# samuelskirvin/EIGENSOLVER

Measured on AMD Instinct MI355X. Metric: det(M) evals/sec + roots/sec, 4096x4096 (k,omega) grid, higher is better.
Workload: dtype f64

## Files before the change

eigensolver_amd/csrc/es_shoot.hip:

```cpp
#include <vector>
#include <cstdio>
#include <cstdlib>
#include <cmath>
#include <type_traits>

#include "es_shoot_shared.hpp"

namespace {
using namespace es_shoot_shared;

struct GridOpts {
  int skip;
  const int* cols;
  int part;
  int main_span;
};

constexpr long ES_TILE_GRID_X = 1L << 22;
__device__ __forceinline__ long es_tile_index() { return (long)blockIdx.y * ES_TILE_GRID_X + blockIdx.x; }
inline dim3 es_tile_grid(long tiles) {
  return tiles <= ES_TILE_GRID_X ? dim3((unsigned)tiles) : dim3((unsigned)ES_TILE_GRID_X, (unsigned)((tiles + ES_TILE_GRID_X - 1) / ES_TILE_GRID_X));
}

template <int FAM, int PTS, int MAXT, bool TRACK, int WPE = 0>
// ... 113 lines not shown
  const int lane = threadIdx.x & 63;
  double d0 = 0.0; int ok0 = 0;
  if (c < cells) { d0 = D[c]; ok0 = (st[c] == ES_PT_OK); }
  double d1 = __shfl_down(d0, 1);
  int ok1 = __shfl_down(ok0, 1);
  if (lane == 63) {
    if (c + 1 < cells) { d1 = D[c + 1]; ok1 = (st[c + 1] == ES_PT_OK); } else { d1 = 0.0; ok1 = 0; }
  }
  bool flag = false;
  if (c < cells) {
    const long row = c / nw;
    const int j = (int)(c - row * nw);
    flag = (j < nw - 1) && ok0 && ok1 && (d0 * d1 < 0.0);
  }
  const uint64_t m = __ballot(flag);
  if (lane == 0) {
    masks[c >> 6] = m;
    wave_cnt[threadIdx.x >> 6] = __popcll(m);
  }
  __syncthreads();
  if (threadIdx.x == 0) block_counts[blockIdx.x] = wave_cnt[0] + wave_cnt[1] + wave_cnt[2] + wave_cnt[3];
}

__global__ __launch_bounds__(256) void bracket_emit_kernel(const double* __restrict__ kv,
                                                           const double* __restrict__ wv, int nw, int w_mode,
                                                           long cells, const double* __restrict__ D,
                                                           const uint64_t* __restrict__ masks,
                                                           const int* __restrict__ block_off, es_root_table tab,
                                                           double* __restrict__ d_lo_sign, double* __restrict__ d_hi_sign) {
  const long c = (long)blockIdx.x * 256 + threadIdx.x;
  if (c >= cells) return;
  const uint64_t m = masks[c >> 6];
  if (!((m >> (c & 63)) & 1ull)) return;
  const int pos = es_cell_rank(masks, block_off, c);
  if (pos >= tab.capacity) return;
  const long row = c / nw;
  const int j = (int)(c - row * nw);
  const double k = kv[row];
  tab.d_k[pos] = k;
  tab.d_row[pos] = (int32_t)row;
  tab.d_w_lo[pos] = pick_w(wv, w_mode, k, (int)row, nw, j);
  tab.d_w_hi[pos] = pick_w(wv, w_mode, k, (int)row, nw, j + 1);
  d_lo_sign[pos] = D[c];
  d_hi_sign[pos] = D[c + 1];
}

constexpr int kRefineSections = 17;
constexpr int kSharedMin = 0;

constexpr int REFINE_WAVES = 4;

template <int FAM, int LANES, int CHR = 0, bool SECTIONS_ONLY = false, bool ONE = false,
          int WPE = ((FAM == FAM_CYLT || !ONE) ? 2 : 3)>
__global__ __launch_bounds__(64 * REFINE_WAVES) __attribute__((amdgpu_waves_per_eu(WPE, WPE)))
void refine_kernel(ShootDev P, es_root_table tab, double* d_lo, double* d_hi, const int* __restrict__ d_n, int n_max,
                   int n_rounds, int n_polish, double tol_percent) {
  const int n = es_count(d_n, n_max);
  if ((int)(blockIdx.x * REFINE_WAVES * (64 / LANES)) >= n) return;
  constexpr int GROUPS = 64 / LANES;
  constexpr int WTBL = GROUPS * (2 * (CHR > 0 ? CHR : 1) + 1) * FamTraits<FAM>::NE;
  __shared__ double es_point_lds[CHR > 0 ? REFINE_WAVES * WTBL : FamTraits<FAM>::NB * (2 * es_shoot_shared::CH + 1)];
  const int lane = threadIdx.x & 63;
  const int g = lane / LANES, j = lane % LANES;
  const int i = (blockIdx.x * REFINE_WAVES + ((int)threadIdx.x >> 6)) * GROUPS + g;
  const bool in = i < n;
  const double k = in ? tab.d_k[i] : 1.0;
  double lo = in ? tab.d_w_lo[i] : 1.0;
  double hi = in ? tab.d_w_hi[i] : 2.0;
  double flo = in ? d_lo[i] : 1.0;
  double fhi = in ? d_hi[i] : -1.0;
  const double frac = (double)(j + 1) / (double)(LANES + 1);
  double D = 0.0, rel = 0.0; uint8_t st = 0;
  double root = lo;
  const int n_final = (n_polish > 0) ? n_polish : (n_polish == 0 ? 1 : 0);
  const int n_it = ONE ? 1 : n_rounds + n_final;
  for (int it = 0; it < n_it; ++it) {
    const bool section = ONE ? true : it < n_rounds;
    double x;
    if (section) {
      x = lo + (hi - lo) * frac;
    } else if (n_polish > 0) {
      x = lo - flo * (hi - lo) / (fhi - flo);
      if (!(x > lo && x < hi)) x = (x == x) ? ((fabs(flo) <= fabs(fhi)) ? lo : hi) : lo + (hi - lo) * 0.5;
    } else {
      x = lo + (hi - lo) * 0.5;
    }
    if (CHR > 0) shoot_point_wavegroup<FAM, (CHR > 0 ? CHR : 1), GROUPS>(P, k, x, D, rel, st, es_point_lds + ((int)threadIdx.x >> 6) * WTBL);
    else if (SECTIONS_ONLY) shoot_point<FAM, false>(P, k, x, x, D, rel, st, es_point_lds);
    else shoot_point<FAM>(P, k, x, x, D, rel, st, es_point_lds);
    if (section) {
      const bool diff = (D * flo < 0.0);
      const unsigned long long bal = __ballot(diff);
      const unsigned long long bits = (LANES == 64) ? bal : ((bal >> (LANES * g)) & ((1ull << (LANES & 63)) - 1ull));
      const int first = bits ? (__ffsll((long long)bits) - 1) : LANES;
      const int src_hi = g * LANES + (first < LANES ? first : LANES - 1);
      const int src_lo = g * LANES + (first > 0 ? first - 1 : 0);
      const double x_hi = __shfl(x, src_hi), d_hi_new = __shfl(D, src_hi);
      const double x_lo = __shfl(x, src_lo), d_lo_new = __shfl(D, src_lo);
      if (first < LANES) { hi = x_hi; fhi = d_hi_new; }
      if (first > 0) { lo = x_lo; flo = (d_lo_new == d_lo_new) ? d_lo_new : flo; }
    } else {
      root = x;
      if (n_polish > 0) {
        if (D * flo < 0.0) { hi = x; fhi = D; } else if (D == D) { lo = x; flo = D; }
      }
    }
  }
  if (in && j == 0) {
    tab.d_w_lo[i] = lo;
    tab.d_w_hi[i] = hi;
    if (n_polish < 0) {
      d_lo[i] = flo;
      d_hi[i] = fhi;
    } else {
      tab.d_w[i] = root;
      tab.d_resid[i] = rel;
      tab.d_flag[i] = (st == ES_PT_OK && rel < tol_percent) ? 1 : 0;
    }
  }
}

template <int FAM, bool ONE = false, int WPE = ((FAM == FAM_CYLT || !ONE) ? 2 : 3)>
__global__ __launch_bounds__(64 * REFINE_WAVES) __attribute__((amdgpu_waves_per_eu(WPE, WPE)))
void refine_polish_kernel(ShootDev P, es_root_table tab, double* d_lo, double* d_hi, const int* __restrict__ d_n,
                          int n_max, int n_polish, double tol_percent) {
  ES_POINT_LDS(FAM);
  const int n = es_count(d_n, n_max);
  if ((int)(blockIdx.x * (64 * REFINE_WAVES)) >= n) return;
  const int i = blockIdx.x * (64 * REFINE_WAVES) + (int)threadIdx.x;
  const bool in = i < n;
  const double k = in ? tab.d_k[i] : 1.0;
  double lo = in ? tab.d_w_lo[i] : 1.0;
  double hi = in ? tab.d_w_hi[i] : 2.0;
  double flo = in ? d_lo[i] : 1.0;
  double fhi = in ? d_hi[i] : -1.0;
  double D = 0.0, rel = 0.0; uint8_t st = 0;
  double root = lo;
  const int n_it = ONE ? 1 : n_polish;
  for (int it = 0; it < n_it; ++it) {
    double x = lo - flo * (hi - lo) / (fhi - flo);
    if (!(x > lo && x < hi)) x = (x == x) ? ((fabs(flo) <= fabs(fhi)) ? lo : hi) : lo + (hi - lo) * 0.5;
    shoot_point<FAM>(P, k, x, x, D, rel, st, es_point_lds);
    root = x;
    if (D * flo < 0.0) { hi = x; fhi = D; } else if (D == D) { lo = x; flo = D; }
  }
  if (in) {
    tab.d_w_lo[i] = lo;
    tab.d_w_hi[i] = hi;
    if (ONE && n_polish == 0) {
      d_lo[i] = flo;
      d_hi[i] = fhi;
    } else {
      tab.d_w[i] = root;
      tab.d_resid[i] = rel;
      tab.d_flag[i] = (st == ES_PT_OK && rel < tol_percent) ? 1 : 0;
    }
  }
}

constexpr int kHybridSections = 1;
constexpr int kHybridSteps = 8;
constexpr double kHybridEps = 1e-12;

struct HybridState {
  double* lo; double* hi; double* flo; double* fhi; double* xprev;
  int* info;
};
constexpr int HYB_ACTIVE = 0, HYB_KEPT = 1, HYB_FAILED = 2;

template <int FAM, int WPE = (FAM == FAM_CYL0 ? 3 : 2)>
__global__ __launch_bounds__(64 * REFINE_WAVES) __attribute__((amdgpu_waves_per_eu(WPE, WPE)))
void refine_superlinear_kernel(ShootDev P, es_root_table tab, const double* d_lo, const double* d_hi, HybridState S,
                               const int* __restrict__ d_n, int n_max, int step, double tol_percent,
                               unsigned long long* stats) {
  ES_POINT_LDS(FAM);
  const int n = es_count(d_n, n_max);
  if ((int)(blockIdx.x * (64 * REFINE_WAVES)) >= n) return;
  const int i = blockIdx.x * (64 * REFINE_WAVES) + (int)threadIdx.x;
  const bool in = i < n;
  const bool first = step == 0;
  const int info = (in && !first) ? S.info[i] : 0;
  const bool active = in && ((info >> 2) == HYB_ACTIVE);
  if (!__syncthreads_or(active ? 1 : 0)) return;
  const double k = in ? tab.d_k[i] : 1.0;
  double lo, hi, flo, fhi, xprev;
  if (first) {
    lo = in ? tab.d_w_lo[i] : 1.0;
    hi = in ? tab.d_w_hi[i] : 2.0;
    flo = in ? d_lo[i] : 1.0;
    fhi = in ? d_hi[i] : -1.0;
    xprev = NAN;
  } else {
    lo = active ? S.lo[i] : 1.0;
    hi = active ? S.hi[i] : 2.0;
    flo = active ? S.flo[i] : 1.0;
    fhi = active ? S.fhi[i] : -1.0;
    xprev = active ? S.xprev[i] : NAN;
  }
  int side = info & 3, status = info >> 2;
  double D = 0.0, rel = 0.0; uint8_t st = 0;
  double x = lo - flo * (hi - lo) / (fhi - flo);
  if (!(x > lo && x < hi)) x = lo + (hi - lo) * 0.5;
  shoot_point<FAM>(P, k, x, x, D, rel, st, es_point_lds);
  if (active) {
    if (D == D) {
      if (D * flo < 0.0) { hi = x; fhi = D; if (side == 1) flo *= 0.5; side = 1; }
      else { lo = x; flo = D; if (side == 2) fhi *= 0.5; side = 2; }
      const double ax = fabs(x);
      if (D == 0.0 || fabs(x - xprev) <= kHybridEps * ax || (hi - lo) <= kHybridEps * ax)
        status = (st == ES_PT_OK && rel < tol_percent) ? HYB_KEPT : HYB_FAILED;
    } else {
      status = HYB_FAILED;
    }
    if (status == HYB_KEPT) {
      tab.d_w_lo[i] = lo;
      tab.d_w_hi[i] = hi;
      tab.d_w[i] = x;
      tab.d_resid[i] = rel;
      tab.d_flag[i] = 1;
    } else if (status == HYB_ACTIVE) {
      S.lo[i] = lo; S.hi[i] = hi; S.flo[i] = flo; S.fhi[i] = fhi; S.xprev[i] = x;
    }
    S.info[i] = side | (status << 2);
  }
  const int n_eval = __popcll(__ballot(active)), n_kept = __popcll(__ballot(active && status == HYB_KEPT));
  if ((threadIdx.x & 63) == 0) {
    if (first && n_eval) atomicAdd(stats + 0, (unsigned long long)n_eval);
    if (n_kept) atomicAdd(stats + 1, (unsigned long long)n_kept);
    if (n_eval) atomicAdd(stats + 3, (unsigned long long)n_eval);
  }
}

__global__ __launch_bounds__(256) void hybrid_flag_kernel(const int* __restrict__ info, const int* __restrict__ d_n,
                                                          int n_max, uint64_t* __restrict__ masks,
                                                          int* __restrict__ block_counts, unsigned long long* stats) {
  __shared__ int wave_cnt[4];
  const int n = es_count(d_n, n_max);
  const int i = blockIdx.x * 256 + (int)threadIdx.x;
  const bool flag = i < n && (info[i] >> 2) != HYB_KEPT;
  const uint64_t m = __ballot(flag);
  if ((threadIdx.x & 63) == 0) {
    masks[i >> 6] = m;
    wave_cnt[threadIdx.x >> 6] = __popcll(m);
  }
  __syncthreads();
  if (threadIdx.x == 0) {
    const int c = wave_cnt[0] + wave_cnt[1] + wave_cnt[2] + wave_cnt[3];
    block_counts[blockIdx.x] = c;
    if (c) atomicAdd(stats + 2, (unsigned long long)c);
  }
}

__global__ __launch_bounds__(256) void hybrid_gather_kernel(es_root_table tab, es_root_table ftab, int* __restrict__ idx,
                                                            const uint64_t* __restrict__ masks,
                                                            const int* __restrict__ block_off,
                                                            const int* __restrict__ d_n, int n_max) {
  const int n = es_count(d_n, n_max);
  const int i = blockIdx.x * 256 + (int)threadIdx.x;
  if (i >= n) return;
  if (!((masks[i >> 6] >> (i & 63)) & 1ull)) return;
  const int pos = es_cell_rank(masks, block_off, (long)i);
  if (pos >= ftab.capacity) return;
  ftab.d_k[pos] = tab.d_k[i];
  ftab.d_w_lo[pos] = tab.d_w_lo[i];
  ftab.d_w_hi[pos] = tab.d_w_hi[i];
  ftab.d_w[pos] = tab.d_w[i];
  ftab.d_resid[pos] = tab.d_resid[i];
  ftab.d_row[pos] = tab.d_row[i];
  idx[pos] = i;
}

__global__ __launch_bounds__(256) void hybrid_scatter_kernel(es_root_table ftab, es_root_table tab,
                                                             const int* __restrict__ idx,
                                                             const int* __restrict__ d_nf, int n_max) {
  const int nf = *d_nf < n_max ? *d_nf : n_max;
  const int j = blockIdx.x * 256 + (int)threadIdx.x;
  if (j >= nf) return;
  const int i = idx[j];
  if (i < 0 || i >= tab.capacity) return;
  tab.d_w[i] = ftab.d_w[j];
  tab.d_w_lo[i] = ftab.d_w_lo[j];
  tab.d_w_hi[i] = ftab.d_w_hi[j];
  tab.d_resid[i] = ftab.d_resid[j];
  tab.d_flag[i] = ftab.d_flag[j];
}

constexpr float F32_TAU_NODE = 1e-3f;
constexpr double F32_TAU_D = 5e-2;
constexpr double F32_TAU_POLE = 5e-2;
constexpr uint8_t F32_UNSURE = 0x80;

typedef float v2f __attribute__((ext_vector_type(2)));

__device__ __forceinline__ v2f v2(float x) { return (v2f){x, x}; }
__device__ __forceinline__ v2f vfma(v2f a, v2f b, v2f c) { return __builtin_elementwise_fma(a, b, c); }
__device__ __forceinline__ v2f vabs(v2f a) { return __builtin_elementwise_abs(a); }
__device__ __forceinline__ v2f vmin(v2f a, v2f b) { return __builtin_elementwise_min(a, b); }
__device__ __forceinline__ v2f vmax(v2f a, v2f b) { return __builtin_elementwise_max(a, b); }
__device__ __forceinline__ v2f vrcp(v2f a) { return (v2f){__builtin_amdgcn_rcpf(a.x), __builtin_amdgcn_rcpf(a.y)}; }

struct CoefF { v2f a11, a12, a21, a22; };
struct CoefPreF { v2f n11, n12, n21, n22, den; };

template <bool TRACK>
struct ScreenF {
  v2f mn = {3.0e38f, 3.0e38f};
// ... 480 lines not shown
GridShape pick_shape(int nw, bool track) {
  GridShape best{4, 2};
  double best_cost = 1e300;
  for (int pts : {4, 3, 2, 1}) {
    if (ShapeTable<FAM>::wpe[pts] == 0) continue;
    const int T = shape_threads(nw, pts);
    const long span = (long)T * pts;
    const long padded = (nw + span - 1) / span * span;
    static const double wave_count_cost[5] = {0.0, 1.83, 1.39, 1.17, 1.0};
    const double c = (double)padded * ShapeTable<FAM>::cost[pts] * wave_count_cost[T / 64];
    if (c < best_cost) { best_cost = c; best = GridShape{pts, ShapeTable<FAM>::wpe[pts]}; }
  }
  if (track && fam_has_bands<FAM>()) best.wpe = 2;
  if (const char* ev = getenv("ES_GRID_SHAPE")) {
    int p = 0, w = 0;
    if (sscanf(ev, "%d,%d", &p, &w) == 2 && p >= 1 && p <= 4 && w >= 2 && w <= 4) best = GridShape{p, w};
  }
  return best;
}

template <int FAM, int PTS, int WPE, bool TRACK>
constexpr bool shape_built() {
  if (PTS == 3 && ShapeTable<FAM>::wpe[3] == 0) return false;
#if defined(ES_ALL_GRID_SHAPES)
  return true;
#else
  if (TRACK && fam_has_bands<FAM>()) return WPE == 2;
  if (FAM == FAM_CYL0 && PTS == 4 && WPE == 2) return true;
  return ShapeTable<FAM>::wpe[PTS] == WPE;
#endif
}

template <int FAM>
bool rows2_shape(int nw, bool track) {
  if (!fam_has_bands<FAM>() || track || nw > 512) return false;
  const char* r2 = getenv("ES_GRID_ROWS2");
  return !(r2 && r2[0] == '0') && !getenv("ES_GRID_SHAPE");
}

template <int FAM>
int launch_grid(es_context* ctx, const es_problem* prob, const double* d_k, int nk, const double* d_w, int nw,
                int w_mode, double* d_D, double* d_rel, uint8_t* d_status, int flags = 0) {
  GridOpts opts;
  opts.skip = (flags & ES_EVAL_SKIP_CONTINUUM) ? 1 : 0;
  opts.cols = nullptr;
  opts.part = 0;
  opts.main_span = 0;
  if (opts.skip && w_mode == ES_W_PHASE_SPEED && fam_has_bands<FAM>() && prob->dev.use_bands) {
    if ((size_t)nw + 1 > ctx->cols_cap) {
      ES_HIP_CHECK(ctx, hipStreamSynchronize(ctx->stream));
      if (ctx->d_cols) ES_HIP_CHECK(ctx, hipFree(ctx->d_cols));
      if (ctx->d_coldead) ES_HIP_CHECK(ctx, hipFree(ctx->d_coldead));
      ctx->d_cols = nullptr; ctx->d_coldead = nullptr; ctx->cols_cap = 0;
      ES_HIP_CHECK(ctx, hipMalloc(&ctx->d_cols, ((size_t)nw + 1) * sizeof(int)));
      ES_HIP_CHECK(ctx, hipMalloc(&ctx->d_coldead, (size_t)nw));
      ctx->cols_cap = (size_t)nw + 1;
    }
    hipLaunchKernelGGL(column_classify_kernel, dim3(1), dim3(1024), 0, ctx->stream, prob->dev, d_w, nw, ctx->d_cols,
                       ctx->d_coldead);
    ES_HIP_CHECK(ctx, hipGetLastError());
    const long cells = (long)nk * nw;
    const int fb = (int)((cells + 255) / 256 < 8192 ? (cells + 255) / 256 : 8192);
    hipLaunchKernelGGL(fill_dead_columns_kernel, dim3(fb), dim3(256), 0, ctx->stream, prob->dev, d_k, nk, d_w, nw,
                       ctx->d_coldead, d_D, d_rel, d_status);
    ES_HIP_CHECK(ctx, hipGetLastError());
    opts.cols = ctx->d_cols;
  }
  const bool track = !(fam_has_bands<FAM>() && prob->dev.use_bands);
  GridShape shape = pick_shape<FAM>(nw, track);
  const int T = shape_threads(nw, shape.pts);
  const long tiles = (long)nk * ((nw + (long)T * shape.pts - 1) / ((long)T * shape.pts));
  const dim3 grid = es_tile_grid(tiles);
  bool launched = false;
  es_timer_begin(ctx);
  if constexpr (fam_has_bands<FAM>()) {
    if (rows2_shape<FAM>(nw, track) && !opts.cols && nk >= 2) {
      const int pts2 = (nw + 127) / 128;
      const dim3 grid2 = es_tile_grid(((long)nk + 1) / 2);
#define ES_R2(P_)                                                                                                   \
      if (pts2 == P_) hipLaunchKernelGGL((shoot_grid_kernel_r2<FAM, P_, false, 3>), grid2, dim3(256), 0, ctx->stream, \
                                         prob->dev, d_k, nk, d_w, nw, w_mode, d_D, d_rel, d_status, opts);
      ES_R2(1) ES_R2(2) ES_R2(3) ES_R2(4)
#undef ES_R2
      launched = true;
    }
  }
  auto one = [&](auto pts_c, auto wpe_c, auto track_c) {
    constexpr int PTS = decltype(pts_c)::value, WPE = decltype(wpe_c)::value;
    constexpr bool TRACK = decltype(track_c)::value;
    if constexpr (shape_built<FAM, PTS, WPE, TRACK>() && (TRACK || fam_has_bands<FAM>())) {
      if (launched || shape.pts != PTS || shape.wpe != WPE || track != TRACK) return;
      launched = true;
      if constexpr (FAM == FAM_CYL0 && PTS == 4 && !TRACK) {
        if (opts.cols && T > 64) {
          opts.part = 1;
          hipLaunchKernelGGL((shoot_grid_kernel<FAM, PTS, 256, TRACK, WPE>), grid, dim3(T), 0, ctx->stream,
                             prob->dev, d_k, nk, d_w, nw, w_mode, d_D, d_rel, d_status, opts);
          opts.part = 2;
          opts.main_span = 4 * T;
          const long tiles2 = (long)nk * (T / 64);
          hipLaunchKernelGGL((shoot_grid_kernel<FAM, 4, 64, false, 2>), es_tile_grid(tiles2),
                             dim3(64), 0, ctx->stream, prob->dev, d_k, nk, d_w, nw, w_mode, d_D, d_rel, d_status, opts);
          return;
        }
      }
      hipLaunchKernelGGL((shoot_grid_kernel<FAM, PTS, 256, TRACK, WPE>), grid, dim3(T), 0, ctx->stream, prob->dev,
                         d_k, nk, d_w, nw, w_mode, d_D, d_rel, d_status, opts);
    }
  };
  using std::integral_constant;
#define ES_SHAPE(P_, W_)                                                                                            \
  one(integral_constant<int, P_>{}, integral_constant<int, W_>{}, integral_constant<bool, false>{});                \
  one(integral_constant<int, P_>{}, integral_constant<int, W_>{}, integral_constant<bool, true>{});
  ES_SHAPE(4, 2) ES_SHAPE(4, 3) ES_SHAPE(4, 4) ES_SHAPE(3, 2) ES_SHAPE(3, 3) ES_SHAPE(2, 2) ES_SHAPE(2, 3) ES_SHAPE(2, 4) ES_SHAPE(1, 2) ES_SHAPE(1, 3) ES_SHAPE(1, 4)
#undef ES_SHAPE
  es_timer_end(ctx);
  if (!launched) {
    ctx->last_error = "grid launch shape not built (ES_GRID_SHAPE names a shape outside this build)";
    return ES_ERR_UNSUPPORTED;
  }
  ES_HIP_CHECK(ctx, hipGetLastError());
  return ES_SUCCESS;
}

inline int es_bound(long n_max) { return (int)(n_max < INT32_MAX ? n_max : INT32_MAX); }
inline dim3 es_blocks(long n_max) { return dim3((unsigned)((n_max + 255) / 256)); }

template <int FAM>
int launch_points(es_context* ctx, const es_problem* prob, const double* d_k, const double* d_w, const int* d_n, long n_max,
                  double* d_D, double* d_rel, uint8_t* d_status) {
  hipLaunchKernelGGL((shoot_points_kernel<FAM>), es_blocks(n_max), dim3(256), 0, ctx->stream, prob->dev, d_k, d_w, d_n,
                     es_bound(n_max), d_D, d_rel, d_status);
  ES_HIP_CHECK(ctx, hipGetLastError());
  return ES_SUCCESS;
}

int dispatch_points(es_context* ctx, const es_problem* prob, const double* d_k, const double* d_w, const int* d_n, long n_max,
                    double* d_D, double* d_rel, uint8_t* d_status) {
#define CALL_PTS(F) launch_points<F>(ctx, prob, d_k, d_w, d_n, n_max, d_D, d_rel, d_status)
  ES_DISPATCH_FAMILY(prob->dev.family, CALL_PTS)
#undef CALL_PTS
}

template <int FAM>
int launch_refine_steps(es_context* ctx, const es_problem* prob, const es_root_table& tab, double* d_lo, double* d_hi,
                        const int* d_n, int n_max, int n_hint, int sections, int rounds, int np, bool polish, double tol) {
  constexpr int CHR = (FAM == FAM_CYL0) ? 32 : 0;
  int shared_min = kSharedMin;
  if (const char* ev = getenv("ES_REFINE_SHARED_MIN")) shared_min = atoi(ev);
  const bool shared_entries = CHR > 0 && np < 0 && n_hint >= shared_min && !getenv("ES_REFINE_PRIVATE_ENTRIES");
  auto blocks = [&](int per_wg) { return dim3((n_max + per_wg - 1) / per_wg); };
  constexpr bool ONE_ROUND_FAM = (FAM == FAM_CYLT || FAM == FAM_CYL0);
  const bool one_round = ONE_ROUND_FAM && !getenv("ES_REFINE_ROUNDS_IN_KERNEL");
#define ES_REFINE(LANES_, CHR_, SO_, PER_WG_)                                                                           \
  if (SO_ && one_round) {                                                                                               \
    if constexpr (ONE_ROUND_FAM && SO_) {                                                                               \
      for (int r_ = 0; r_ < rounds; ++r_)                                                                               \
        hipLaunchKernelGGL((refine_kernel<FAM, LANES_, CHR_, true, true>), blocks(PER_WG_), dim3(64 * REFINE_WAVES), 0, \
                           ctx->stream, prob->dev, tab, d_lo, d_hi, d_n, n_max, 1, np, tol);                            \
    }                                                                                                                   \
  } else                                                                                                                \
    hipLaunchKernelGGL((refine_kernel<FAM, LANES_, CHR_, SO_, false>), blocks(PER_WG_), dim3(64 * REFINE_WAVES), 0,     \
                       ctx->stream, prob->dev, tab, d_lo, d_hi, d_n, n_max, rounds, np, tol)
  if (sections == 17 && shared_entries) ES_REFINE(16, CHR, true, 4 * REFINE_WAVES);
  else if (np < 0) {
    if (sections == 17) ES_REFINE(16, 0, true, 4 * REFINE_WAVES);
    else if (sections == 9) ES_REFINE(8, 0, true, 8 * REFINE_WAVES);
    else ES_REFINE(4, 0, true, 16 * REFINE_WAVES);
  } else {
    if (sections == 17) ES_REFINE(16, 0, false, 4 * REFINE_WAVES);
    else if (sections == 9) ES_REFINE(8, 0, false, 8 * REFINE_WAVES);
    else ES_REFINE(4, 0, false, 16 * REFINE_WAVES);
  }
#undef ES_REFINE
  ES_HIP_CHECK(ctx, hipGetLastError());
  if (np < 0 && polish) {
    if (one_round) {
      if constexpr (ONE_ROUND_FAM) {
        for (int p_ = 0; p_ < ES_REFINE_POLISH; ++p_)
          hipLaunchKernelGGL((refine_polish_kernel<FAM, true>), blocks(64 * REFINE_WAVES), dim3(64 * REFINE_WAVES), 0, ctx->stream,
                             prob->dev, tab, d_lo, d_hi, d_n, n_max, p_ == ES_REFINE_POLISH - 1 ? 1 : 0, tol);
      }
    } else
      hipLaunchKernelGGL((refine_polish_kernel<FAM, false>), blocks(64 * REFINE_WAVES), dim3(64 * REFINE_WAVES), 0, ctx->stream,
                         prob->dev, tab, d_lo, d_hi, d_n, n_max, ES_REFINE_POLISH, tol);
    ES_HIP_CHECK(ctx, hipGetLastError());
  }
  return ES_SUCCESS;
}

int refine_sections() {
  int sections = kRefineSections;
  if (const char* ev = getenv("ES_REFINE_SECTIONS")) {
    const int v = atoi(ev);
    if (v == 5 || v == 9 || v == 17) sections = v;
  }
  return sections;
}

int check_refine_rule(es_context* ctx) {
  if (ctx->refine_rule == ES_REFINE_HYBRID && refine_sections() != kRefineSections) {
    ctx->last_error = "ES_REFINE_HYBRID is defined for 17-section only (ES_REFINE_SECTIONS is set to another rule)";
    return ES_ERR_UNSUPPORTED;
  }
  return ES_SUCCESS;
}

template <int FAM>
int launch_refine_hybrid(es_context* ctx, const es_problem* prob, const es_root_table& tab, const int* d_n, int n_max,
                         int n_hint, int rounds, double tol) {
  if (n_max <= 0) return ES_SUCCESS;
  auto align = [](size_t b) { return (b + 255) & ~(size_t)255; };
  const size_t cap = (size_t)n_max;
  const size_t bd = align(cap * sizeof(double)), bi = align(cap * sizeof(int)), bf = align(cap);
  const int nblk = (n_max + 255) / 256;
  const size_t bm = align((size_t)nblk * 4 * sizeof(uint64_t)), bc = align((size_t)(nblk + 1) * sizeof(int));
  int rc = es_ensure_hybrid_scratch(ctx, 10 * bd + 3 * bi + bf + bm + bc + 256);
  if (rc) return rc;
  char* b = (char*)ctx->d_hybrid;
  auto take = [&](size_t bytes) { char* p = b; b += bytes; return p; };
  HybridState S;
  S.lo = (double*)take(bd); S.hi = (double*)take(bd); S.flo = (double*)take(bd); S.fhi = (double*)take(bd);
  S.xprev = (double*)take(bd);
  S.info = (int*)take(bi);
  es_root_table ftab;
  ftab.d_k = (double*)take(bd); ftab.d_w = (double*)take(bd); ftab.d_w_lo = (double*)take(bd);
  ftab.d_w_hi = (double*)take(bd); ftab.d_resid = (double*)take(bd);
  ftab.d_row = (int32_t*)take(bi); ftab.d_flag = (uint8_t*)take(bf);
  ftab.capacity = n_max;
  int* idx = (int*)take(bi);
  uint64_t* masks = (uint64_t*)take(bm);
  int* counts = (int*)take(bc);
  int* d_nf = (int*)take(256);
  rc = launch_refine_steps<FAM>(ctx, prob, tab, tab.d_w, tab.d_resid, d_n, n_max, n_hint, kRefineSections, kHybridSections,
                                -1, false, tol);
  if (rc) return rc;
  const dim3 wg(64 * REFINE_WAVES), grid((n_max + 64 * REFINE_WAVES - 1) / (64 * REFINE_WAVES));
  for (int s_ = 0; s_ < kHybridSteps; ++s_)
    hipLaunchKernelGGL((refine_superlinear_kernel<FAM>), grid, wg, 0, ctx->stream, prob->dev, tab, tab.d_w, tab.d_resid, S,
                       d_n, n_max, s_, tol, ctx->d_refine_stats);
  ES_HIP_CHECK(ctx, hipGetLastError());
  hipLaunchKernelGGL(hybrid_flag_kernel, dim3(nblk), dim3(256), 0, ctx->stream, S.info, d_n, n_max, masks, counts,
                     ctx->d_refine_stats);
  ES_HIP_CHECK(ctx, hipGetLastError());
  rc = es_scan_counts_async(ctx, counts, nblk, d_nf);
  if (rc) return rc;
  hipLaunchKernelGGL(hybrid_gather_kernel, dim3(nblk), dim3(256), 0, ctx->stream, tab, ftab, idx, masks, counts, d_n, n_max);
  ES_HIP_CHECK(ctx, hipGetLastError());
  rc = launch_refine_steps<FAM>(ctx, prob, ftab, ftab.d_w, ftab.d_resid, d_nf, n_max, n_hint, kRefineSections,
                                rounds - kHybridSections, -1, true, tol);
  if (rc) return rc;
  hipLaunchKernelGGL(hybrid_scatter_kernel, dim3(nblk), dim3(256), 0, ctx->stream, ftab, tab, idx, d_nf, n_max);
  ES_HIP_CHECK(ctx, hipGetLastError());
  return ES_SUCCESS;
}

template <int FAM>
int launch_refine(es_context* ctx, const es_problem* prob, const es_root_table& tab, double* d_lo, double* d_hi,
                  const int* d_n, int n_max, int n_hint, int n_bisect, double tol) {
  const int sections = refine_sections();
  int rounds = 0;
  for (double span = 1.0, need = ldexp(1.0, n_bisect < 1000 ? n_bisect : 1000); span < need; span *= (double)sections) ++rounds;
  if (ctx->refine_rule == ES_REFINE_HYBRID) {
    const int rc = check_refine_rule(ctx);
    if (rc) return rc;
    if (rounds > kHybridSections) return launch_refine_hybrid<FAM>(ctx, prob, tab, d_n, n_max, n_hint, rounds, tol);
  }
  const int np = (ES_REFINE_POLISH > 0 && rounds > 0) ? -1 : ES_REFINE_POLISH;
  return launch_refine_steps<FAM>(ctx, prob, tab, d_lo, d_hi, d_n, n_max, n_hint, sections, rounds, np, true, tol);
}

int dispatch_refine(es_context* ctx, const es_problem* prob, const es_root_table& tab, const int* d_n, int n_max, int n_hint,
                    int n_bisect, double tol) {
#define CALL_REFINE(F) launch_refine<F>(ctx, prob, tab, tab.d_w, tab.d_resid, d_n, n_max, n_hint, n_bisect, tol)
  ES_DISPATCH_FAMILY(prob->dev.family, CALL_REFINE)
#undef CALL_REFINE
}

}

extern "C" int es_problem_create(es_context* ctx, const es_shoot_desc* d, const es_profiles* pr, es_problem** out) {
  if (!ctx) return ES_ERR_INVALID_ARG;
  ES_REQUIRE(ctx, d && pr && out, "null pointer");
  *out = nullptr;
  ES_REQUIRE(ctx, d->n_nodes >= 2 && d->n_nodes <= (1 << 24), "n_nodes out of range");
  ES_REQUIRE(ctx, d->geometry >= 0 && d->geometry <= 3, "geometry");
  ES_REQUIRE(ctx, d->x_boundary == -1.0 || d->x_boundary == 1.0, "x_boundary must be -1 or +1");
  const int N = d->n_nodes, npts = 2 * N - 1;
  int nb = 0;
  switch (d->geometry) {
    case ES_GEOM_CYLINDER: nb = FamTraits<FAM_CYL0>::NB; break;
    case ES_GEOM_CYLINDER_TWIST: nb = FamTraits<FAM_CYLT>::NB; break;
    case ES_GEOM_SLAB_DENSITY: nb = FamTraits<FAM_SLABD>::NB; break;
    default: nb = FamTraits<FAM_SLABF>::NB; break;
  }
  std::vector<double> base((size_t)nb * npts);
  auto B = [&](int f, int i) -> double& { return base[(size_t)f * npts + i]; };
  if (d->geometry == ES_GEOM_CYLINDER || d->geometry == ES_GEOM_CYLINDER_TWIST) {
    ES_REQUIRE(ctx, pr->r && pr->rho && pr->c2 && pr->Bz, "cylinder profiles r, rho, c2, Bz required");
    ES_REQUIRE(ctx, d->axis_bc >= 0 && d->axis_bc <= 2, "axis_bc");
    ES_REQUIRE(ctx, d->c1_power == 1 || d->c1_power == 2, "c1_power");
    ES_REQUIRE(ctx, d->m >= 0 && d->m_ext >= 0 && d->m_ext <= 64, "m");
    for (int i = 0; i < npts; ++i) {
      const double r = pr->r[i], rho = pr->rho[i], c2 = pr->c2[i], Bz = pr->Bz[i];
      const double Bphi = pr->Bphi ? pr->Bphi[i] : 0.0;
      const double vz = pr->vz ? pr->vz[i] : 0.0;
      const double vphi = pr->vphi ? pr->vphi[i] : 0.0;
      const double sr = sqrt(rho);
      const double bA = Bz / sr;
      const double vA = (Bz + Bphi) / sr;
      const double S = c2 + vA * vA;
      const double q = c2 / S;
      if (d->geometry == ES_GEOM_CYLINDER) {
        ES_REQUIRE(ctx, Bphi == 0.0 && vphi == 0.0, "ES_GEOM_CYLINDER needs Bphi = vphi = 0 (use CYLINDER_TWIST)");
        B(C0_VZ, i) = vz;
        B(C0_BA, i) = bA;
        B(C0_Q, i) = q;
        B(C0_A1, i) = rho / r;
        B(C0_B1, i) = r / (rho * S);
        B(C0_E1, i) = 1.0 / (r * rho);
        B(C0_E2, i) = r / rho;
      } else {
        const double dm = (double)d->m, dm2 = dm * dm;
        const double invr = 1.0 / r, invr2 = invr * invr;
        const double bphr = Bphi / r, vphr = vphi / r;
        const double Bphi_n = bphr * r, vphi_n = vphr * r;
        B(CT_MB, i) = dm * bphr;
        B(CT_BZ, i) = Bz;
        B(CT_BA, i) = bA;
        B(CT_MV, i) = dm * vphr;
        B(CT_VZ, i) = vz;
// ... 593 lines not shown
```

eigensolver_amd/csrc/es_shoot_shared.hpp:

```cpp
#pragma once
#include "es_common.hpp"
#include "es_shoot_device.hpp"

struct es_problem {
  ShootDev dev;
  double* d_base = nullptr;
  es_shoot_desc desc;
};

namespace es_shoot_shared {

constexpr int ES_REFINE_POLISH = 2;
#if defined(ES_STAGE_FAR_NODE_ALWAYS)
#define ES_FAR_NODE(c_, n_) 1
#else
#define ES_FAR_NODE(c_, n_) (((c_) == (n_) - 1) ? 1 : 0)
#endif
constexpr int CH = 128;

template <int FAM>
__device__ __forceinline__ void load_base(const ShootDev& P, int pt, double* b) {
#pragma unroll
  for (int f = 0; f < FamTraits<FAM>::NB; ++f) b[f] = P.base[(size_t)f * P.npts + pt];
}
// ... 88 lines not shown
          Coef Nm, N1, Nm2, N2;
          ES_ENTRY(2 * j - 3, e)
          ES_ENTRY(2 * j - 4, e1)
          ES_ENTRY(2 * j - 5, em2)
          ES_ENTRY(2 * j - 6, e2)
          coefficients4<FAM, TRACK>(e, e1, em2, e2, P, s, w, Nm, N1, Nm2, N2, trk);
          adjoint_step<FAM>(zp, zq, B0, Cm, C1, h, h2, h6, h3);
          adjoint_step<FAM>(zp, zq, C1, Cm2, C2, h, h2, h6, h3);
          B0 = C2;
          Cm = Nm; C1 = N1; Cm2 = Nm2; C2 = N2;
        }
        adjoint_step<FAM>(zp, zq, B0, Cm, C1, h, h2, h6, h3);
        adjoint_step<FAM>(zp, zq, C1, Cm2, C2, h, h2, h6, h3);
        B0 = C2;
      }
    } else {
      Coef Cm, C1;
      ES_ENTRY(2 * j + 1, e)
      ES_ENTRY(2 * j, e2)
      coefficients2<FAM, TRACK, C1P>(e, e2, P, s, w, Cm, C1, trk);
      for (; j >= 1; --j) {
        Coef Nm, N1;
        ES_ENTRY(2 * j - 1, e)
        ES_ENTRY(2 * j - 2, e2)
        coefficients2<FAM, TRACK, C1P>(e, e2, P, s, w, Nm, N1, trk);
        adjoint_step<FAM>(zp, zq, B0, Cm, C1, h, h2, h6, h3);
        B0 = C1;
        Cm = Nm; C1 = N1;
      }
      adjoint_step<FAM>(zp, zq, B0, Cm, C1, h, h2, h6, h3);
      B0 = C1;
    }
#undef ES_ENTRY
    adjoint_rescale<FAM>(zp, zq, nsteps - c0 - nst, nsteps - c0);
  }
  const Mismatch M = boundary_algebra<FAM>(P, s, w, X, zp, zq, e2);
  finish_point(P, M, X, TRACK ? trk.crossed() : (BANDS ? band_crossed(P, k, w) : false), D, rel, st);
}

template <int FAM, bool TRACK, int CHR, int NG>
__device__ __forceinline__ void shoot_point_wavegroup_impl(const ShootDev& P, double k, double w, double& D, double& rel,
                                                           uint8_t& st, double* __restrict__ tbl) {
  constexpr int NE = FamTraits<FAM>::NE;
  constexpr int NB = FamTraits<FAM>::NB;
  constexpr int NODES = 2 * CHR + 1;
  constexpr int GL = 64 / NG;
  const int lane = threadIdx.x & 63;
  const int grp = lane / GL;
  const KScal s = make_kscal(P, k);
  const int nsteps = P.n_nodes - 1;
  const double h = P.h, h2 = 0.5 * P.h, h6 = P.h / 6.0, h3 = P.h / 3.0;
  SignTrack trk;
  double e[NE], e2[NE];
  const ExteriorLite X = exterior_lite(P, k, w, w);
  Coef B0;
  double zp = 0.0, zq = 0.0;
  const double* mine = tbl + (size_t)grp * NODES * NE;
  double kgs[NG];
#pragma unroll
  for (int g2 = 0; g2 < NG; ++g2) kgs[g2] = __shfl(k, g2 * GL);
  const int nchunks = (nsteps + CHR - 1) / CHR;
  for (int c = nchunks - 1; c >= 0; --c) {
    const int c0 = c * CHR;
    const int nst = (nsteps - c0 < CHR) ? (nsteps - c0) : CHR;
    const int nn = 2 * nst + ES_FAR_NODE(c, nchunks);
    __builtin_amdgcn_wave_barrier();
    for (int idx = lane; idx < NG * nn; idx += 64) {
      const int g2 = idx / nn, i = idx - g2 * nn;
      double kg = kgs[0];
#pragma unroll
      for (int q = 1; q < NG; ++q) kg = (g2 == q) ? kgs[q] : kg;
      const KScal sg = make_kscal(P, kg);
      double b[NB], eg[NE];
#pragma unroll
      for (int f = 0; f < NB; ++f) b[f] = P.base[(size_t)f * P.npts + 2 * c0 + i];
      make_entry<FAM, fam_scaled<FAM>()>(b, sg, eg);
#pragma unroll
      for (int f = 0; f < NE; ++f) tbl[((size_t)g2 * NODES + i) * NE + f] = eg[f];
    }
    __builtin_amdgcn_wave_barrier();
    if (c == nchunks - 1) {
#pragma unroll
      for (int f = 0; f < NE; ++f) e[f] = mine[2 * nst * NE + f];
      coefficients<FAM, TRACK>(e, P, s, w, B0, trk);
      adjoint_start(P, B0, zp, zq);
    }
    int j = nst - 1;
    if (!fam_rcp4<FAM>() || !(j & 1)) {
      for (; j >= 0 && (!fam_rcp4<FAM>() || !(j & 1)); --j) {
        Coef Bm, B1;
#pragma unroll
        for (int f = 0; f < NE; ++f) { e[f] = mine[(2 * j + 1) * NE + f]; e2[f] = mine[2 * j * NE + f]; }
        coefficients2<FAM, TRACK>(e, e2, P, s, w, Bm, B1, trk);
        adjoint_step<FAM>(zp, zq, B0, Bm, B1, h, h2, h6, h3);
        B0 = B1;
      }
    }
    if (fam_rcp4<FAM>() && j >= 1) {
      double e1[NE], em2[NE];
      Coef Cm, C1, Cm2, C2;
#pragma unroll
      for (int f = 0; f < NE; ++f) {
        e[f] = mine[(2 * j + 1) * NE + f]; e1[f] = mine[2 * j * NE + f];
        em2[f] = mine[(2 * j - 1) * NE + f]; e2[f] = mine[(2 * j - 2) * NE + f];
      }
      coefficients4<FAM, TRACK>(e, e1, em2, e2, P, s, w, Cm, C1, Cm2, C2, trk);
      for (; j >= 3; j -= 2) {
        Coef Nm, N1, Nm2, N2;
#pragma unroll
        for (int f = 0; f < NE; ++f) {
          e[f] = mine[(2 * j - 3) * NE + f]; e1[f] = mine[(2 * j - 4) * NE + f];
          em2[f] = mine[(2 * j - 5) * NE + f]; e2[f] = mine[(2 * j - 6) * NE + f];
        }
        coefficients4<FAM, TRACK>(e, e1, em2, e2, P, s, w, Nm, N1, Nm2, N2, trk);
        adjoint_step<FAM>(zp, zq, B0, Cm, C1, h, h2, h6, h3);
        adjoint_step<FAM>(zp, zq, C1, Cm2, C2, h, h2, h6, h3);
        B0 = C2;
        Cm = Nm; C1 = N1; Cm2 = Nm2; C2 = N2;
      }
      adjoint_step<FAM>(zp, zq, B0, Cm, C1, h, h2, h6, h3);
      adjoint_step<FAM>(zp, zq, C1, Cm2, C2, h, h2, h6, h3);
      B0 = C2;
    }
    adjoint_rescale<FAM>(zp, zq, nsteps - c0 - nst, nsteps - c0);
  }
  const Mismatch M = boundary_algebra<FAM>(P, s, w, X, zp, zq, e2);
  finish_point(P, M, X, TRACK ? trk.crossed() : band_crossed(P, k, w), D, rel, st);
}

template <int FAM, int CHR, int NG>
__device__ __forceinline__ void shoot_point_wavegroup(const ShootDev& P, double k, double w, double& D, double& rel,
                                                      uint8_t& st, double* __restrict__ tbl) {
  if (fam_has_bands<FAM>() && P.use_bands) shoot_point_wavegroup_impl<FAM, !fam_has_bands<FAM>(), CHR, NG>(P, k, w, D, rel, st, tbl);
  else shoot_point_wavegroup_impl<FAM, true, CHR, NG>(P, k, w, D, rel, st, tbl);
}

template <int FAM, bool STATUS = true>
__device__ __forceinline__ void shoot_point(const ShootDev& P, double k, double w, double w_cst, double& D,
                                            double& rel, uint8_t& st, double* __restrict__ sb) {
  if (FAM == FAM_CYLT) {
    if (!STATUS) {
      if (P.c1_power == 2) shoot_point_impl<FAM, false, false, 2>(P, k, w, w_cst, D, rel, st, sb);
      else shoot_point_impl<FAM, false, false, 1>(P, k, w, w_cst, D, rel, st, sb);
    } else {
      if (P.c1_power == 2) shoot_point_impl<FAM, true, false, 2>(P, k, w, w_cst, D, rel, st, sb);
      else shoot_point_impl<FAM, true, false, 1>(P, k, w, w_cst, D, rel, st, sb);
    }
  } else if (!STATUS) {
    shoot_point_impl<FAM, false, false>(P, k, w, w_cst, D, rel, st, sb);
  } else if (fam_has_bands<FAM>() && P.use_bands) shoot_point_impl<FAM, !fam_has_bands<FAM>()>(P, k, w, w_cst, D, rel, st, sb);
  else shoot_point_impl<FAM, true>(P, k, w, w_cst, D, rel, st, sb);
}

#define ES_POINT_LDS(FAM) __shared__ double es_point_lds[FamTraits<FAM>::NB * (2 * es_shoot_shared::CH + 1)]

}
```

Before: 855.2 million.

## Add copy-free paired-march refine and secant kernels for CYL0 family

For the CYL0 family, the per-round refine and polish launches now go to new kernels. These use a paired adjoint march with double-buffered coefficient sets (coefficients4, steps unrolled by four) and read node entries directly from a wave-shared LDS table rather than copying them into private arrays. The round kernel brackets the sign change using a ballot and shuffle across the section lanes. The aim is to cut register and copy overhead in the shooting march. In exchange there is more code and register pressure, and bracket selection and rescaling may differ slightly from the legacy path.

```diff
diff --git a/eigensolver_amd/csrc/es_shoot.hip b/eigensolver_amd/csrc/es_shoot.hip
--- a/eigensolver_amd/csrc/es_shoot.hip
+++ b/eigensolver_amd/csrc/es_shoot.hip
@@ -289,6 +289,88 @@
       d_hi[i] = fhi;
     } else {
       tab.d_w[i] = root;
+      tab.d_resid[i] = rel;
+      tab.d_flag[i] = (st == ES_PT_OK && rel < tol_percent) ? 1 : 0;
+    }
+  }
+}
+
+template <int FAM, int LANES, int CHR, int WPE = 3>
+__global__ __launch_bounds__(64 * REFINE_WAVES) __attribute__((amdgpu_waves_per_eu(WPE, WPE)))
+void section_round_kernel(ShootDev P, es_root_table tab, double* d_lo, double* d_hi, const int* __restrict__ d_n, int n_max) {
+  static_assert(CHR > 0 && 64 % LANES == 0 && LANES < 64, "wave-shared node entries");
+  const int n = es_count(d_n, n_max);
+  if ((int)(blockIdx.x * REFINE_WAVES * (64 / LANES)) >= n) return;
+  constexpr int GROUPS = 64 / LANES;
+  constexpr int WTBL = GROUPS * (2 * CHR + 1) * FamTraits<FAM>::NE;
+  __shared__ double es_point_lds[REFINE_WAVES * WTBL];
+  const int lane = threadIdx.x & 63;
+  const int g = lane / LANES, j = lane % LANES;
+  const int i = (blockIdx.x * REFINE_WAVES + ((int)threadIdx.x >> 6)) * GROUPS + g;
+  const bool in = i < n;
+  const double k = in ? tab.d_k[i] : 1.0;
+  double x;
+  {
+    const double lo0 = in ? tab.d_w_lo[i] : 1.0, hi0 = in ? tab.d_w_hi[i] : 2.0;
+    x = lo0 + (hi0 - lo0) * ((double)(j + 1) / (double)(LANES + 1));
+  }
+  double D = 0.0, rel = 0.0; uint8_t st = 0;
+  shoot_point_wavegroup_impl2<FAM, false, CHR, GROUPS>(P, k, x, D, rel, st, es_point_lds + ((int)threadIdx.x >> 6) * WTBL);
+  __asm__ volatile("" ::: "memory");
+  double lo = in ? tab.d_w_lo[i] : 1.0;
+  double hi = in ? tab.d_w_hi[i] : 2.0;
+  double flo = in ? d_lo[i] : 1.0;
+  double fhi = in ? d_hi[i] : -1.0;
+  const bool diff = (D * flo < 0.0);
+  const unsigned long long bal = __ballot(diff);
+  const unsigned long long bits = (bal >> (LANES * g)) & ((1ull << LANES) - 1ull);
+  const int first = bits ? (__ffsll((long long)bits) - 1) : LANES;
+  const int src_hi = g * LANES + (first < LANES ? first : LANES - 1);
+  const int src_lo = g * LANES + (first > 0 ? first - 1 : 0);
+  const double x_hi = __shfl(x, src_hi), d_hi_new = __shfl(D, src_hi);
+  const double x_lo = __shfl(x, src_lo), d_lo_new = __shfl(D, src_lo);
+  if (first < LANES) { hi = x_hi; fhi = d_hi_new; }
+  if (first > 0) { lo = x_lo; flo = (d_lo_new == d_lo_new) ? d_lo_new : flo; }
+  if (in && j == 0) {
+    tab.d_w_lo[i] = lo;
+    tab.d_w_hi[i] = hi;
+    d_lo[i] = flo;
+    d_hi[i] = fhi;
+  }
+}
+
+template <int FAM, int WPE = 3>
+__global__ __launch_bounds__(64 * REFINE_WAVES) __attribute__((amdgpu_waves_per_eu(WPE, WPE)))
+void secant_step_kernel(ShootDev P, es_root_table tab, double* d_lo, double* d_hi, const int* __restrict__ d_n, int n_max,
+                        int last, double tol_percent) {
+  ES_POINT_LDS(FAM);
+  const int n = es_count(d_n, n_max);
+  if ((int)(blockIdx.x * (64 * REFINE_WAVES)) >= n) return;
+  const int i = blockIdx.x * (64 * REFINE_WAVES) + (int)threadIdx.x;
+  const bool in = i < n;
+  const double k = in ? tab.d_k[i] : 1.0;
+  double lo = in ? tab.d_w_lo[i] : 1.0;
+  double hi = in ? tab.d_w_hi[i] : 2.0;
+  double flo = in ? d_lo[i] : 1.0;
+  double fhi = in ? d_hi[i] : -1.0;
+  double D = 0.0, rel = 0.0; uint8_t st = 0;
+  double x = lo - flo * (hi - lo) / (fhi - flo);
+  if (!(x > lo && x < hi)) x = (x == x) ? ((fabs(flo) <= fabs(fhi)) ? lo : hi) : lo + (hi - lo) * 0.5;
+  shoot_point2<FAM>(P, k, x, x, D, rel, st, es_point_lds);
+  __asm__ volatile("" ::: "memory");
+  lo = in ? tab.d_w_lo[i] : 1.0;
+  hi = in ? tab.d_w_hi[i] : 2.0;
+  flo = in ? d_lo[i] : 1.0;
+  fhi = in ? d_hi[i] : -1.0;
+  if (D * flo < 0.0) { hi = x; fhi = D; } else if (D == D) { lo = x; flo = D; }
+  if (in) {
+    tab.d_w_lo[i] = lo;
+    tab.d_w_hi[i] = hi;
+    if (!last) {
+      d_lo[i] = flo;
+      d_hi[i] = fhi;
+    } else {
+      tab.d_w[i] = x;
       tab.d_resid[i] = rel;
       tab.d_flag[i] = (st == ES_PT_OK && rel < tol_percent) ? 1 : 0;
     }
@@ -1075,9 +1157,20 @@
   auto blocks = [&](int per_wg) { return dim3((n_max + per_wg - 1) / per_wg); };
   constexpr bool ONE_ROUND_FAM = (FAM == FAM_CYLT || FAM == FAM_CYL0);
   const bool one_round = ONE_ROUND_FAM && !getenv("ES_REFINE_ROUNDS_IN_KERNEL");
+  constexpr bool COPY_FREE_FAM = (FAM == FAM_CYL0);
+  const char* march_ev = getenv("ES_REFINE_MARCH");
+  const bool copy_free = COPY_FREE_FAM && one_round && !(march_ev && !strcmp(march_ev, "legacy"));
 #define ES_REFINE(LANES_, CHR_, SO_, PER_WG_)                                                                           \
   if (SO_ && one_round) {                                                                                               \
-    if constexpr (ONE_ROUND_FAM && SO_) {                                                                               \
+    if constexpr (COPY_FREE_FAM && SO_ && CHR_ > 0) {                                                                   \
+      for (int r_ = 0; r_ < rounds; ++r_)                                                                               \
+        if (copy_free)                                                                                                  \
+          hipLaunchKernelGGL((section_round_kernel<FAM, LANES_, CHR_>), blocks(PER_WG_), dim3(64 * REFINE_WAVES), 0,    \
+                             ctx->stream, prob->dev, tab, d_lo, d_hi, d_n, n_max);                                      \
+        else                                                                                                            \
+          hipLaunchKernelGGL((refine_kernel<FAM, LANES_, CHR_, true, true>), blocks(PER_WG_), dim3(64 * REFINE_WAVES),  \
+                             0, ctx->stream, prob->dev, tab, d_lo, d_hi, d_n, n_max, 1, np, tol);                       \
+    } else if constexpr (ONE_ROUND_FAM && SO_) {                                                                        \
       for (int r_ = 0; r_ < rounds; ++r_)                                                                               \
         hipLaunchKernelGGL((refine_kernel<FAM, LANES_, CHR_, true, true>), blocks(PER_WG_), dim3(64 * REFINE_WAVES), 0, \
                            ctx->stream, prob->dev, tab, d_lo, d_hi, d_n, n_max, 1, np, tol);                            \
@@ -1099,7 +1192,15 @@
   ES_HIP_CHECK(ctx, hipGetLastError());
   if (np < 0 && polish) {
     if (one_round) {
-      if constexpr (ONE_ROUND_FAM) {
+      if constexpr (COPY_FREE_FAM) {
+        for (int p_ = 0; p_ < ES_REFINE_POLISH; ++p_)
+          if (copy_free)
+            hipLaunchKernelGGL((secant_step_kernel<FAM>), blocks(64 * REFINE_WAVES), dim3(64 * REFINE_WAVES), 0, ctx->stream,
+                               prob->dev, tab, d_lo, d_hi, d_n, n_max, p_ == ES_REFINE_POLISH - 1 ? 1 : 0, tol);
+          else
+            hipLaunchKernelGGL((refine_polish_kernel<FAM, true>), blocks(64 * REFINE_WAVES), dim3(64 * REFINE_WAVES), 0, ctx->stream,
+                               prob->dev, tab, d_lo, d_hi, d_n, n_max, p_ == ES_REFINE_POLISH - 1 ? 1 : 0, tol);
+      } else if constexpr (ONE_ROUND_FAM) {
         for (int p_ = 0; p_ < ES_REFINE_POLISH; ++p_)
           hipLaunchKernelGGL((refine_polish_kernel<FAM, true>), blocks(64 * REFINE_WAVES), dim3(64 * REFINE_WAVES), 0, ctx->stream,
                              prob->dev, tab, d_lo, d_hi, d_n, n_max, p_ == ES_REFINE_POLISH - 1 ? 1 : 0, tol);
diff --git a/eigensolver_amd/csrc/es_shoot_shared.hpp b/eigensolver_amd/csrc/es_shoot_shared.hpp
--- a/eigensolver_amd/csrc/es_shoot_shared.hpp
+++ b/eigensolver_amd/csrc/es_shoot_shared.hpp
@@ -264,6 +264,183 @@
   else shoot_point_impl<FAM, true>(P, k, w, w_cst, D, rel, st, sb);
 }
 
+#define ES_PAIRED_MARCH(LOAD4)                                                                 \
+  if (j >= 1) {                                                                                \
+    double e1[NE], em2[NE];                                                                    \
+    Coef Am, A1, Am2, A2, Bm, B1, Bm2, B2;                                                     \
+    LOAD4(j)                                                                                   \
+    coefficients4<FAM, TRACK>(e, e1, em2, e2, P, s, w, Am, A1, Am2, A2, trk);                  \
+    if (((j + 1) >> 1) & 1) {                           \
+      if (j >= 3) {                                                                            \
+        LOAD4(j - 2)                                                                           \
+        coefficients4<FAM, TRACK>(e, e1, em2, e2, P, s, w, Bm, B1, Bm2, B2, trk);              \
+      }                                                                                        \
+      adjoint_step<FAM>(zp, zq, B0, Am, A1, h, h2, h6, h3);                                    \
+      adjoint_step<FAM>(zp, zq, A1, Am2, A2, h, h2, h6, h3);                                   \
+      B0 = A2;                                                                                 \
+      if (j >= 3) { Am = Bm; A1 = B1; Am2 = Bm2; A2 = B2; }    \
+      j -= 2;                                                                                  \
+    }                                                                                          \
+    for (; j >= 7; j -= 4) {                            \
+      LOAD4(j - 2)                                                                             \
+      coefficients4<FAM, TRACK>(e, e1, em2, e2, P, s, w, Bm, B1, Bm2, B2, trk);                \
+      adjoint_step<FAM>(zp, zq, B0, Am, A1, h, h2, h6, h3);                                    \
+      adjoint_step<FAM>(zp, zq, A1, Am2, A2, h, h2, h6, h3);                                   \
+      B0 = A2;                                                                                 \
+      LOAD4(j - 4)                                                                             \
+      coefficients4<FAM, TRACK>(e, e1, em2, e2, P, s, w, Am, A1, Am2, A2, trk);                \
+      adjoint_step<FAM>(zp, zq, B0, Bm, B1, h, h2, h6, h3);                                    \
+      adjoint_step<FAM>(zp, zq, B1, Bm2, B2, h, h2, h6, h3);                                   \
+      B0 = B2;                                                                                 \
+    }                                                                                          \
+    if (j >= 3) {                                                      \
+      LOAD4(j - 2)                                                                             \
+      coefficients4<FAM, TRACK>(e, e1, em2, e2, P, s, w, Bm, B1, Bm2, B2, trk);                \
+      adjoint_step<FAM>(zp, zq, B0, Am, A1, h, h2, h6, h3);                                    \
+      adjoint_step<FAM>(zp, zq, A1, Am2, A2, h, h2, h6, h3);                                   \
+      adjoint_step<FAM>(zp, zq, A2, Bm, B1, h, h2, h6, h3);                                    \
+      adjoint_step<FAM>(zp, zq, B1, Bm2, B2, h, h2, h6, h3);                                   \
+      B0 = B2;                                                                                 \
+    }                                                                                          \
+  }
+
+template <int FAM, bool TRACK, bool BANDS = !TRACK>
+__device__ __forceinline__ void shoot_point_impl2(const ShootDev& P, double k, double w, double w_cst, double& D,
+                                                  double& rel, uint8_t& st, double* __restrict__ sb) {
+  static_assert(fam_rcp4<FAM>(), "paired marches only");
+  constexpr int NE = FamTraits<FAM>::NE;
+  constexpr int NB = FamTraits<FAM>::NB;
+  const KScal s = make_kscal(P, k);
+  const int nsteps = P.n_nodes - 1;
+  const double h = P.h, h2 = 0.5 * P.h, h6 = P.h / 6.0, h3 = P.h / 3.0;
+  SignTrack trk;
+  double b[NB], e[NE], e2[NE];
+  const ExteriorLite X = exterior_lite(P, k, w, w_cst);
+  Coef B0;
+  double zp = 0.0, zq = 0.0;
+  const int nchunks = (nsteps + CH - 1) / CH;
+  for (int c = nchunks - 1; c >= 0; --c) {
+    const int c0 = c * CH;
+    const int nst = (nsteps - c0 < CH) ? (nsteps - c0) : CH;
+    __syncthreads();
+#pragma unroll
+    for (int f = 0; f < NB; ++f)
+      for (int i = threadIdx.x; i < 2 * nst + ES_FAR_NODE(c, nchunks); i += blockDim.x)
+        sb[i * NB + f] = P.base[(size_t)f * P.npts + 2 * c0 + i];
+    __syncthreads();
+#define ES_ENTRY(NODE, E)                                                                      \
+    {                                                                                          \
+      _Pragma("unroll") for (int f = 0; f < NB; ++f) b[f] = sb[(NODE) * NB + f];               \
+      make_entry<FAM, fam_scaled<FAM>()>(b, s, E);                                             \
+    }
+#define ES_ENTRY4(J) ES_ENTRY(2 * (J) + 1, e) ES_ENTRY(2 * (J), e1) ES_ENTRY(2 * (J) - 1, em2) ES_ENTRY(2 * (J) - 2, e2)
+    if (c == nchunks - 1) {
+      ES_ENTRY(2 * nst, e)
+      coefficients<FAM, TRACK>(e, P, s, w, B0, trk);
+      adjoint_start(P, B0, zp, zq);
+    }
+    int j = nst - 1;
+    if (!(j & 1)) {
+      Coef Bm, B1;
+      ES_ENTRY(2 * j + 1, e)
+      ES_ENTRY(2 * j, e2)
+      coefficients2<FAM, TRACK>(e, e2, P, s, w, Bm, B1, trk);
+      adjoint_step<FAM>(zp, zq, B0, Bm, B1, h, h2, h6, h3);
+      B0 = B1;
+      --j;
+    }
+    ES_PAIRED_MARCH(ES_ENTRY4)
+#undef ES_ENTRY4
+#undef ES_ENTRY
+    adjoint_rescale<FAM>(zp, zq, nsteps - c0 - nst, nsteps - c0);
+  }
+  const Mismatch M = boundary_algebra<FAM>(P, s, w, X, zp, zq, e2);
+  finish_point(P, M, X, TRACK ? trk.crossed() : (BANDS ? band_crossed(P, k, w) : false), D, rel, st);
+}
+
+template <int FAM, bool TRACK, int CHR, int NG>
+__device__ __forceinline__ void shoot_point_wavegroup_impl2(const ShootDev& P, double k, double w, double& D, double& rel,
+                                                            uint8_t& st, double* __restrict__ tbl) {
+  static_assert(fam_rcp4<FAM>() && CHR % 2 == 0, "paired marches only");
+  constexpr int NE = FamTraits<FAM>::NE;
+  constexpr int NB = FamTraits<FAM>::NB;
+  constexpr int NODES = 2 * CHR + 1;
+  constexpr int GL = 64 / NG;
+  const int lane = threadIdx.x & 63;
+  const int grp = lane / GL;
+  const KScal s = make_kscal(P, k);
+  const int nsteps = P.n_nodes - 1;
+  const double h = P.h, h2 = 0.5 * P.h, h6 = P.h / 6.0, h3 = P.h / 3.0;
+  SignTrack trk;
+  double e[NE], e2[NE];
+  Coef B0;
+  double zp = 0.0, zq = 0.0;
+  const double* mine = tbl + (size_t)grp * NODES * NE;
+  double kgs[NG];
+#pragma unroll
+  for (int g2 = 0; g2 < NG; ++g2)
+    kgs[g2] = __hiloint2double(__builtin_amdgcn_readlane(__double2hiint(k), g2 * GL),
+                               __builtin_amdgcn_readlane(__double2loint(k), g2 * GL));
+  const int nchunks = (nsteps + CHR - 1) / CHR;
+  for (int c = nchunks - 1; c >= 0; --c) {
+    const int c0 = c * CHR;
+    const int nst = (nsteps - c0 < CHR) ? (nsteps - c0) : CHR;
+    const int nn = 2 * nst + ES_FAR_NODE(c, nchunks);
+    __builtin_amdgcn_wave_barrier();
+    KScal sgs[NG];
+#pragma unroll
+    for (int g2 = 0; g2 < NG; ++g2) sgs[g2] = make_kscal(P, kgs[g2]);
+    for (int i = lane; i < nn; i += 64) {
+      double b[NB];
+#pragma unroll
+      for (int f = 0; f < NB; ++f) b[f] = P.base[(size_t)f * P.npts + 2 * c0 + i];
+#pragma unroll
+      for (int g2 = 0; g2 < NG; ++g2) {
+        double eg[NE];
+        make_entry<FAM, fam_scaled<FAM>()>(b, sgs[g2], eg);
+#pragma unroll
+        for (int f = 0; f < NE; ++f) tbl[((size_t)g2 * NODES + i) * NE + f] = eg[f];
+      }
+    }
+    __builtin_amdgcn_wave_barrier();
+#define ES_TABLE4(J)                                                                           \
+    _Pragma("unroll") for (int f = 0; f < NE; ++f) {                                           \
+      e[f] = mine[(2 * (J) + 1) * NE + f]; e1[f] = mine[2 * (J) * NE + f];                     \
+      em2[f] = mine[(2 * (J) - 1) * NE + f]; e2[f] = mine[(2 * (J) - 2) * NE + f];             \
+    }
+    if (c == nchunks - 1) {
+#pragma unroll
+      for (int f = 0; f < NE; ++f) e[f] = mine[2 * nst * NE + f];
+      coefficients<FAM, TRACK>(e, P, s, w, B0, trk);
+      adjoint_start(P, B0, zp, zq);
+    }
+    int j = nst - 1;
+    if (!(j & 1)) {
+      Coef Bm, B1;
+#pragma unroll
+      for (int f = 0; f < NE; ++f) { e[f] = mine[(2 * j + 1) * NE + f]; e2[f] = mine[2 * j * NE + f]; }
+      coefficients2<FAM, TRACK>(e, e2, P, s, w, Bm, B1, trk);
+      adjoint_step<FAM>(zp, zq, B0, Bm, B1, h, h2, h6, h3);
+      B0 = B1;
+      --j;
+    }
+    ES_PAIRED_MARCH(ES_TABLE4)
+#undef ES_TABLE4
+    adjoint_rescale<FAM>(zp, zq, nsteps - c0 - nst, nsteps - c0);
+  }
+  const ExteriorLite X = exterior_lite(P, k, w, w);
+  const Mismatch M = boundary_algebra<FAM>(P, s, w, X, zp, zq, e2);
+  finish_point(P, M, X, TRACK ? trk.crossed() : band_crossed(P, k, w), D, rel, st);
+}
+#undef ES_PAIRED_MARCH
+
+template <int FAM>
+__device__ __forceinline__ void shoot_point2(const ShootDev& P, double k, double w, double w_cst, double& D, double& rel,
+                                             uint8_t& st, double* __restrict__ sb) {
+  if (fam_has_bands<FAM>() && P.use_bands) shoot_point_impl2<FAM, !fam_has_bands<FAM>()>(P, k, w, w_cst, D, rel, st, sb);
+  else shoot_point_impl2<FAM, true>(P, k, w, w_cst, D, rel, st, sb);
+}
+
 #define ES_POINT_LDS(FAM) __shared__ double es_point_lds[FamTraits<FAM>::NB * (2 * es_shoot_shared::CH + 1)]
 
 }
```

Result: no change. 858.7 million (median of 6 runs) (+0.4%).
